# submission2019/cnn-quantization

Measured on NVIDIA H100. Metric: resnet50_w4a4_images_per_s, higher is better.
Workload: dtype f32

## Files before the change

### cnn-quantization_b200/csrc/fq_cl.cuh

```cuda
#pragma once

namespace fqb {

__device__ __forceinline__ unsigned enc_ordered(float x) {
  const unsigned b = __float_as_uint(x);
  return (b & 0x80000000u) ? ~b : (b | 0x80000000u);
}
__device__ __forceinline__ float dec_ordered(unsigned e) {
  return __uint_as_float((e & 0x80000000u) ? (e & 0x7fffffffu) : ~e);
}

constexpr unsigned kAccU = 2u * kMaxNhwcChannels;
constexpr unsigned kAccD = 3u * kMaxNhwcChannels;

struct ClView {
  unsigned* amin_inv;
  unsigned* amax;
  double* asum;
  double* asq;
  double* aabs;
};
__device__ __forceinline__ ClView cl_view(const FusedArgs& A, unsigned bank) {
  ClView v;
  v.amin_inv = A.amin_inv + bank * kAccU;
  v.amax = v.amin_inv + kMaxNhwcChannels;
  v.asum = A.asum + bank * kAccD;
  v.asq = v.asum + kMaxNhwcChannels;
  v.aabs = v.asq + kMaxNhwcChannels;
  return v;
}

__device__ __forceinline__ void red_add_f64(double* p, double v) {
  asm volatile("red.global.add.f64 [%0], %1;" ::"l"(p), "d"(v) : "memory");
}
__device__ __forceinline__ void red_max_u32(unsigned* p, unsigned v) {
  asm volatile("red.global.max.u32 [%0], %1;" ::"l"(p), "r"(v) : "memory");
}

__device__ __noinline__ void grid_arrive_cl(GridSync* gs, unsigned& epoch) {
  ++epoch;
  consumer_sync();
  if (threadIdx.x == 0) {
    unsigned prev;
    asm volatile("atom.add.acq_rel.gpu.global.u32 %0, [%1], 1;" : "=r"(prev) : "l"(&gs->arrive) : "memory");
    if (prev + 1u == epoch * gridDim.x) st_release_u32(&gs->release, epoch);
  }
}
__device__ __noinline__ void grid_wait_cl(GridSync* gs, unsigned epoch) {
  if (threadIdx.x == 0) {
    while (ld_acquire_u32(&gs->release) < epoch) __nanosleep(32);
  }
  consumer_sync();
}
__device__ __forceinline__ void grid_barrier_cl(GridSync* gs, unsigned& epoch) {
  grid_arrive_cl(gs, epoch);
  grid_wait_cl(gs, epoch);
}
__device__ __forceinline__ void grid_exit_cl(GridSync* gs) {
  consumer_sync();
  if (threadIdx.x == 0) {
    const unsigned prev = atomicAdd(&gs->exited, 1u);
    if (prev + 1u == gridDim.x) {
      gs->arrive = 0u;
      gs->release = 0u;
      for (int i = 0; i < 8; ++i) gs->unit_counter[i] = 0u;
      gs->launch_count = gs->launch_count + 1u;
      __threadfence();
      gs->exited = 0u;
    }
  }
}

constexpr unsigned kClChunkStages = 1;

struct ClStats1 {
  float mn[4], mx[4], k[4], fs[4], fq[4];
  double s[4], q[4];
  unsigned cnt;
  __device__ __forceinline__ void init(const FusedArgs& A, unsigned c0, bool active) {
    float4 first = make_float4(0.f, 0.f, 0.f, 0.f);
    if (active) first = ld_tensor(reinterpret_cast<const float4*>(A.in) + (c0 >> 2));
    k[0] = first.x;
    k[1] = first.y;
    k[2] = first.z;
    k[3] = first.w;
    cnt = 0;
#pragma unroll
    for (int i = 0; i < 4; ++i) {
      mn[i] = INFINITY;
      mx[i] = -INFINITY;
      fs[i] = 0.f;
      fq[i] = 0.f;
      s[i] = 0.0;
      q[i] = 0.0;
    }
  }
  __device__ __forceinline__ void flush() {
#pragma unroll
    for (int i = 0; i < 4; ++i) {
      s[i] += static_cast<double>(fs[i]);
      q[i] += static_cast<double>(fq[i]);
      fs[i] = 0.f;
      fq[i] = 0.f;
    }
    cnt = 0;
  }
  __device__ __forceinline__ void consume(const float4& v, unsigned) {
    const float x[4] = {v.x, v.y, v.z, v.w};
#pragma unroll
    for (int i = 0; i < 4; ++i) {
      const float d = __fsub_rn(x[i], k[i]);
      mn[i] = fminf(mn[i], x[i]);
      mx[i] = fmaxf(mx[i], x[i]);
      fs[i] = __fadd_rn(fs[i], d);
      fq[i] = __fmaf_rn(d, d, fq[i]);
    }
  }
  __device__ __forceinline__ void stage_end(const StageMeta&) {
    if (++cnt == kClChunkStages) flush();
  }
};

struct ClStats2 {
  float mu[4], bias[4], fa[4];
  double sa[4];
  unsigned cnt;
  __device__ __forceinline__ void init(const FusedArgs& A, unsigned c0, bool active, const float (&mean)[4]) {
    cnt = 0;
#pragma unroll
    for (int i = 0; i < 4; ++i) {
      bias[i] = (A.bias && active) ? __ldg(A.bias + c0 + i) : 0.f;
      mu[i] = mean[i];
      fa[i] = 0.f;
      sa[i] = 0.0;
    }
  }
  __device__ __forceinline__ void flush() {
#pragma unroll
    for (int i = 0; i < 4; ++i) {
      sa[i] += static_cast<double>(fa[i]);
      fa[i] = 0.f;
    }
    cnt = 0;
  }
  __device__ __forceinline__ void consume(const float4& v, unsigned) {
    const float x[4] = {v.x, v.y, v.z, v.w};
#pragma unroll
    for (int i = 0; i < 4; ++i) fa[i] = __fadd_rn(fa[i], fabsf(__fsub_rn(__fadd_rn(x[i], bias[i]), mu[i])));
  }
  __device__ __forceinline__ void stage_end(const StageMeta&) {
    if (++cnt == kClChunkStages) flush();
  }
};

constexpr unsigned kHistWords = 8192;
static_assert(kHistWords * 4u <= kStageBytes, "the histogram borrows one ring stage");

template <int LEAF, bool HIST>
struct ClApply {
  const FusedArgs& A;
  unsigned* hist;
  LeafParam q[4];
  float r[4], bias[4];
  unsigned nlo[4], nhi[4];
  unsigned hbase;
  bool fast;
  LeafParam rq[4];
  float rr[4], rbias[4];
  bool rquant;
  __device__ __forceinline__ void init(unsigned c0, bool active, const LeafParam (&lp)[4]) {
    fast = true;
    rquant = A.residual != nullptr && A.residual_stats != nullptr;
#pragma unroll
    for (int i = 0; i < 4; ++i) {
      rq[i].a = 1.f;
      rq[i].b = 0.f;
      rq[i].c = 0.f;
      rq[i].flags = 0;
      rr[i] = 1.f;
      rbias[i] = 0.f;
      if (rquant && active) {
        const float* row = A.residual_stats + static_cast<size_t>(c0 + i) * FQB200_STATS_STRIDE;
        rq[i].a = __ldg(row + 8);
        rq[i].b = __ldg(row + 9);
        rq[i].c = __ldg(row + 10);
        rq[i].flags = static_cast<int>(__ldg(row + 11));
        const Divisor dr = make_divisor(rq[i].a);
        rr[i] = dr.r;
        fast = fast && dr.fast;
        if (A.residual_bias) rbias[i] = __ldg(A.residual_bias + c0 + i);
      }
    }
    const unsigned copies = max(1u, min(static_cast<unsigned>(kWarps), kHistWords / static_cast<unsigned>(max(A.hist_bins, 1))));
    hbase = ((threadIdx.x >> 5) % copies) * static_cast<unsigned>(A.hist_bins);
#pragma unroll
    for (int i = 0; i < 4; ++i) {
      q[i] = lp[i];
      const Divisor dv = make_divisor(q[i].a);
      r[i] = dv.r;
      fast = fast && dv.fast;
      bias[i] = (A.bias && active) ? __ldg(A.bias + c0 + i) : 0.f;
      nlo[i] = 0u;
      nhi[i] = 0u;
    }
  }
  __device__ __forceinline__ void count(int i, float gq) {
    if (LEAF == FQB200_LEAF_MIDTREAD) {
      if (gq == q[i].c) {
        ++nhi[i];
        return;
      }
      if (gq == q[i].b) {
        ++nlo[i];
        return;
      }
    }
    if (gq == gq) {
      const float v = fminf(fmaxf(gq + static_cast<float>(A.hist_offset), 0.f), static_cast<float>(A.hist_bins - 1));
      atomicAdd(hist + hbase + static_cast<unsigned>(v), 1u);
    }
  }
  template <bool FAST, bool PAIR, bool RQ = false>
  __device__ __forceinline__ void one(const float4& v, const float4& rv, unsigned off) {
    const float x[4] = {v.x, v.y, v.z, v.w};
    float y[4], gq[4];
#pragma unroll
    for (int i = 0; i < 4; ++i) {
      Divisor dv;
      dv.s = q[i].a;
      dv.r = r[i];
      dv.fast = FAST;
      y[i] = leaf_apply<LEAF, FAST>(__fadd_rn(x[i], bias[i]), q[i], dv, 0.f, gq[i]);
    }
    if (PAIR) {
      float res[4] = {rv.x, rv.y, rv.z, rv.w};
      if (RQ) {
#pragma unroll
        for (int i = 0; i < 4; ++i) {
          Divisor dr;
          dr.s = rq[i].a;
          dr.r = rr[i];
          dr.fast = FAST;
          float g2;
          res[i] = leaf_apply<LEAF, FAST>(__fadd_rn(res[i], rbias[i]), rq[i], dr, 0.f, g2);
        }
      }
#pragma unroll
      for (int i = 0; i < 4; ++i) {
        y[i] = __fadd_rn(y[i], res[i]);
        if (A.residual_relu) y[i] = y[i] < 0.f ? 0.f : y[i];
      }
    }
    st_tensor(reinterpret_cast<float4*>(A.out) + off, make_float4(y[0], y[1], y[2], y[3]));
    if (HIST) {
#pragma unroll
      for (int i = 0; i < 4; ++i) count(i, gq[i]);
    }
  }
  __device__ __forceinline__ void consume(const float4& v, unsigned off) {
    if (fast)
      one<true, false>(v, v, off);
    else
      one<false, false>(v, v, off);
  }
  template <bool FAST>
  __device__ __forceinline__ void pooled_one(const float4& a0, const float4& a1, const float4& b0, const float4& b1, unsigned off) {
    auto mx = [](float p, float q) { return (q > p || q != q) ? q : p; };
    const float m[4] = {mx(mx(mx(a0.x, a1.x), b0.x), b1.x), mx(mx(mx(a0.y, a1.y), b0.y), b1.y),
                        mx(mx(mx(a0.z, a1.z), b0.z), b1.z), mx(mx(mx(a0.w, a1.w), b0.w), b1.w)};
    float y[4], gq;
#pragma unroll
    for (int i = 0; i < 4; ++i) {
      Divisor dv;
      dv.s = q[i].a;
      dv.r = r[i];
      dv.fast = FAST;
      y[i] = leaf_apply<LEAF, FAST>(__fadd_rn(m[i], bias[i]), q[i], dv, 0.f, gq);
    }
    st_tensor(reinterpret_cast<float4*>(A.pool_out) + off, make_float4(y[0], y[1], y[2], y[3]));
  }
  __device__ __forceinline__ void pooled(const float4& a0, const float4& a1, const float4& b0, const float4& b1, unsigned off) {
    if (fast)
      pooled_one<true>(a0, a1, b0, b1, off);
    else
      pooled_one<false>(a0, a1, b0, b1, off);
  }
  float pm[4];
  __device__ __forceinline__ void pool_begin() {
#pragma unroll
    for (int i = 0; i < 4; ++i) pm[i] = -INFINITY;
  }
  __device__ __forceinline__ void pool_tap(const float4& v) {
    auto mx = [](float p, float q) { return (q > p || q != q) ? q : p; };
    pm[0] = mx(pm[0], v.x);
    pm[1] = mx(pm[1], v.y);
    pm[2] = mx(pm[2], v.z);
    pm[3] = mx(pm[3], v.w);
  }
  template <bool FAST>
  __device__ __forceinline__ void pool_end_one(unsigned off) {
    float y[4], gq;
#pragma unroll
    for (int i = 0; i < 4; ++i) {
      Divisor dv;
      dv.s = q[i].a;
      dv.r = r[i];
      dv.fast = FAST;
      y[i] = leaf_apply<LEAF, FAST>(__fadd_rn(pm[i], bias[i]), q[i], dv, 0.f, gq);
    }
    st_tensor(reinterpret_cast<float4*>(A.pool_out) + off, make_float4(y[0], y[1], y[2], y[3]));
  }
  __device__ __forceinline__ void pool_end(unsigned off) {
    if (fast)
      pool_end_one<true>(off);
    else
      pool_end_one<false>(off);
  }
  __device__ __forceinline__ void consume2(const float4& v, const float4& rv, unsigned off) {
    if (rquant) {
      if (fast)
        one<true, true, true>(v, rv, off);
      else
        one<false, true, true>(v, rv, off);
    } else if (fast) {
      one<true, true>(v, rv, off);
    } else {
      one<false, true>(v, rv, off);
    }
  }
  __device__ __forceinline__ void stage_end(const StageMeta&) {}
};

constexpr unsigned kClItems = 4;

template <typename T, typename Op>
__device__ __forceinline__ void cl_stage_round(unsigned char* buf, unsigned cv, unsigned stride, const T (&v)[4], T identity, Op op,
                                               T (&res)[kClItems]) {
  T* st = reinterpret_cast<T*>(buf);
  consumer_sync();
#pragma unroll
  for (int i = 0; i < 4; ++i) st[i * kConsumers + threadIdx.x] = (threadIdx.x < stride) ? v[i] : identity;
  consumer_sync();
#pragma unroll
  for (unsigned k = 0; k < kClItems; ++k) {
    const unsigned it = threadIdx.x + k * kConsumers;
    T a = identity;
    if (it < 4u * cv) {
      const unsigned col = it % cv, i = it / cv;
      for (unsigned t = col; t < stride; t += cv) a = op(a, st[i * kConsumers + t]);
    }
    res[k] = a;
  }
}

__device__ __noinline__ void cl_combine_s1(unsigned char* buf, unsigned cv, unsigned stride, const unsigned (&umn)[4],
                                           const unsigned (&umx)[4], const double (&s)[4], const double (&q)[4], unsigned* dmn,
                                           unsigned* dmx, double* ds, double* dq) {
  if (cv == stride) {
    if (threadIdx.x < stride) {
#pragma unroll
      for (int i = 0; i < 4; ++i) {
        const unsigned c = 4u * threadIdx.x + i;
        red_max_u32(dmn + c, umn[i]);
        red_max_u32(dmx + c, umx[i]);
        red_add_f64(ds + c, s[i]);
        red_add_f64(dq + c, q[i]);
      }
    }
    return;
  }
  uint2 mm[4], rmm[kClItems];
#pragma unroll
  for (int i = 0; i < 4; ++i) mm[i] = make_uint2(umn[i], umx[i]);
  auto max2 = [](uint2 a, uint2 b) { return make_uint2(a.x > b.x ? a.x : b.x, a.y > b.y ? a.y : b.y); };
  double rs[kClItems], rq[kClItems];
  cl_stage_round(buf, cv, stride, mm, make_uint2(0u, 0u), max2, rmm);
  cl_stage_round(buf, cv, stride, s, 0.0, OpAdd(), rs);
  cl_stage_round(buf, cv, stride, q, 0.0, OpAdd(), rq);
#pragma unroll
  for (unsigned k = 0; k < kClItems; ++k) {
    const unsigned it = threadIdx.x + k * kConsumers;
    if (it < 4u * cv) {
      const unsigned c = 4u * (it % cv) + it / cv;
      red_max_u32(dmn + c, rmm[k].x);
      red_max_u32(dmx + c, rmm[k].y);
      red_add_f64(ds + c, rs[k]);
      red_add_f64(dq + c, rq[k]);
    }
  }
}
__device__ __noinline__ void cl_combine_add_f64(unsigned char* buf, unsigned cv, unsigned stride, const double (&v0)[4], double* d0,
                                                const double (&v1)[4], double* d1, const double (&v2)[4], double* d2) {
  if (cv == stride) {
    if (threadIdx.x < stride) {
#pragma unroll
      for (int i = 0; i < 4; ++i) {
        const unsigned c = 4u * threadIdx.x + i;
        red_add_f64(d0 + c, v0[i]);
        if (d1) red_add_f64(d1 + c, v1[i]);
        if (d2) red_add_f64(d2 + c, v2[i]);
      }
    }
    return;
  }
  double r0[kClItems], r1[kClItems], r2[kClItems];
  cl_stage_round(buf, cv, stride, v0, 0.0, OpAdd(), r0);
// ... 86 lines not shown
      A.gprior[c] = p;
      local += static_cast<double>(p);
    }
    const float psum = static_cast<float>(block_reduce(local, OpAdd(), sm.d));
    const float budget = static_cast<float>(static_cast<double>(C) * exp2(static_cast<double>(A.mt_target)));
    for (unsigned c = threadIdx.x; c < C; c += kConsumers) A.gbits[c] = rintf(__fdiv_rn(__fmul_rn(budget, A.gprior[c]), psum));
  } else {
    solve_bit_alloc(A, sm);
  }
  consumer_sync();
  if (publish && threadIdx.x == 0) st_release_u32(&A.sync->aux_ready, tag);
}

template <int LEAF, bool DEV>
__device__ __noinline__ LeafParam cl_channel_param(const FusedArgs& A, const ClView& acc, unsigned rep, unsigned C, unsigned c,
                                                   float mu, double n, bool alloc, bool do_export) {
  auto umax = [](unsigned a, unsigned b) { return a > b ? a : b; };
  const unsigned lo = cl_rep_reduce(acc.amin_inv, rep, C, c, 0u, umax);
  const unsigned hi = cl_rep_reduce(acc.amax, rep, C, c, 0u, umax);
  const double sa = DEV ? cl_rep_reduce(acc.aabs, rep, C, c, 0.0, OpAdd()) : 0.0;
  const float cb = A.bias ? __ldg(A.bias + c) : 0.f;
  const float mn = __fadd_rn(dec_ordered(~lo), cb), mx = __fadd_rn(dec_ordered(hi), cb);
  const float b = DEV ? static_cast<float>(sa / n) : 0.f;
  const bool need_sd = A.range_mode == FQB200_RANGE_GAUS || A.range_mode == FQB200_RANGE_KSTD || do_export;
  const float sd = need_sd ? cl_std(acc, rep, C, c, n) : 0.f;
  const float aux = alloc ? ld_ws(A.gbits + c) : static_cast<float>(A.num_bits);
  LeafParam q;
  if constexpr (LEAF == FQB200_LEAF_MIDTREAD) {
    float rng;
    q = mid_tread_param(A, aux, mn, mx, mu, b, rng);
    if (do_export) export_stats(A, c, mn, mx, mu, b, sd, rng, 0.f, aux, q);
  } else {
    float delta, offset;
    solve_range(A, mn, mx, mu, b, sd, aux, delta, offset);
    q = make_leaf_param(LEAF, delta, offset, aux);
    if (do_export) export_stats(A, c, mn, mx, mu, b, sd, delta, offset, aux, q);
  }
  return q;
}

struct ClCtx {
  const FlatGeo* g;
  BulkRing* ring;
  unsigned char* stages;
  unsigned char* cbuf;
  RingPos pos;
  ClView acc;
  unsigned rep_base, c0;
  bool active;
};

__device__ __noinline__ void cl_phase_s1(const FusedArgs& A, ClCtx& cx, float (&kshift)[4]) {
  const FlatGeo& g = *cx.g;
  ClStats1 s1;
  s1.init(A, cx.c0, cx.active);
#pragma unroll
  for (int i = 0; i < 4; ++i) kshift[i] = s1.k[i];
  RingPos pos = cx.pos;
  consume_phase(g, *cx.ring, cx.stages, pos, s1);
  cx.pos = pos;
  s1.flush();
  if (blockIdx.x == 0) stamp(A, 13);
  unsigned umn[4], umx[4];
#pragma unroll
  for (int i = 0; i < 4; ++i) {
    umn[i] = ~enc_ordered(s1.mn[i]);
    umx[i] = enc_ordered(s1.mx[i]);
  }
  const ClView& acc = cx.acc;
  const unsigned rb = cx.rep_base;
  cl_combine_s1(cx.cbuf, g.cv, g.stride, umn, umx, s1.s, s1.q, acc.amin_inv + rb, acc.amax + rb, acc.asum + rb, acc.asq + rb);
}

__device__ __noinline__ void cl_phase_s2(const FusedArgs& A, ClCtx& cx, const float (&mean)[4]) {
  const FlatGeo& g = *cx.g;
  ClStats2 s2;
  s2.init(A, cx.c0, cx.active, mean);
  RingPos pos = cx.pos;
  consume_phase(g, *cx.ring, cx.stages, pos, s2);
  cx.pos = pos;
  s2.flush();
  if (blockIdx.x == 0) stamp(A, 14);
  const ClView& acc = cx.acc;
  const unsigned rb = cx.rep_base;
  cl_combine_add_f64(cx.cbuf, g.cv, g.stride, s2.sa, acc.aabs + rb, s2.sa, nullptr, s2.sa, nullptr);
}

template <int LEAF, bool HIST>
__device__ __noinline__ void cl_phase_apply(const FusedArgs& A, ClCtx& cx, const LeafParam (&lp)[4], unsigned* hist) {
  const FlatGeo& g = *cx.g;
  const unsigned t = threadIdx.x;
  if (HIST) {
    for (unsigned i = t; i < kHistWords; i += kConsumers) hist[i] = 0u;
    consumer_sync();
  }
  ClApply<LEAF, HIST> ap{A, hist};
  ap.init(cx.c0, cx.active, lp);
  RingPos pos = cx.pos;
  if (A.pool.tiles) {
    if (A.pool.kind == 3u)
      consume_pool3_phase(g, A.pool, *cx.ring, cx.stages, pos, ap);
    else
      consume_pool_phase(g, A.pool, *cx.ring, cx.stages, pos, ap);
  } else if (A.residual) {
    const FlatGeo h = half_geo(g);
    consume_pair_phase(h, *cx.ring, cx.stages, pos, ap);
  } else {
    consume_phase(g, *cx.ring, cx.stages, pos, ap);
  }
  cx.pos = pos;
  if (HIST) {
    consumer_sync();
    const unsigned bins = static_cast<unsigned>(A.hist_bins);
    const unsigned copies = max(1u, min(static_cast<unsigned>(kWarps), kHistWords / bins));
    for (unsigned b = t; b < bins; b += kConsumers) {
      unsigned long long cnt = 0;
      for (unsigned w = 0; w < copies; ++w) cnt += hist[w * bins + b];
      if (cnt) atomicAdd(A.hist + b, cnt);
    }
    if (LEAF == FQB200_LEAF_MIDTREAD && A.hist_clamped && cx.active) {
#pragma unroll
      for (int i = 0; i < 4; ++i) {
        if (ap.nlo[i]) atomicAdd(A.hist_clamped + 2u * (cx.c0 + i), static_cast<unsigned long long>(ap.nlo[i]));
        if (ap.nhi[i]) atomicAdd(A.hist_clamped + 2u * (cx.c0 + i) + 1u, static_cast<unsigned long long>(ap.nhi[i]));
      }
    }
  }
}

constexpr unsigned kClStagingBytes = 4u * kConsumers * 8u;
constexpr unsigned kClTableChannels = 1024;
constexpr unsigned kClCombineBytes = kClStagingBytes + kClTableChannels * 4u;

template <int LEAF, bool DEV, bool HIST>
__global__ void __launch_bounds__(kBulkThreads, kBulkCtasPerSm) fq_cl_kernel(const __grid_constant__ FusedArgs A) {
  extern __shared__ __align__(128) unsigned char fq_dyn[];
  unsigned char* stages = fq_dyn;
  unsigned char* cbuf = fq_dyn + kStages * kStageBytes;
  float* tab_mean = reinterpret_cast<float*>(cbuf + kClStagingBytes);
  unsigned* hist = reinterpret_cast<unsigned*>(stages + (kStages - 1) * kStageBytes);
  __shared__ BulkRing ring;
  __shared__ LeaderSmem lsm;
  __shared__ alignas(8) unsigned long long solver_done;
  const FlatGeo& g = A.flat;
  const unsigned C = g.channels, cv = g.cv;
  const unsigned launch = ld_ws(&A.sync->launch_count);
  const unsigned bank = launch & 1u;
  const unsigned tag = launch + 1u;
  const bool alloc = (LEAF == FQB200_LEAF_MIDTREAD) || (A.bit_alloc && A.num_bits <= 4);
  const bool aux_needs_b = alloc && LEAF != FQB200_LEAF_MIDTREAD && A.prior == FQB200_PRIOR_B;
  const bool solver_in_s2 = alloc && !aux_needs_b && DEV && gridDim.x > 1u;
  __shared__ alignas(8) unsigned long long phase_go[2];
  if (threadIdx.x == 0) {
    mbar_init(smem_u32(&solver_done), 1u);
    mbar_init(smem_u32(&phase_go[0]), 1u);
    mbar_init(smem_u32(&phase_go[1]), 1u);
  }
  const unsigned nstages = HIST ? kStages - 1u : kStages;
  ring_init(ring, nstages);

  if (threadIdx.x >= kConsumers) {
    if (threadIdx.x == kConsumers) {
      RingPos pos;
      pos.init(nstages);
      const float4* src = reinterpret_cast<const float4*>(A.in);
      const TicketPlan all = {2u, blockIdx.x, gridDim.x, 2u * gridDim.x};
      const TicketPlan no0 = {blockIdx.x == 0 ? 0u : 2u, blockIdx.x - 1u, gridDim.x - 1u, 2u * (gridDim.x - 1u)};
      produce_phase<false>(g, src, &A.sync->unit_counter[0], all, ring, stages, pos);
      if (DEV) {
        mbar_wait(smem_u32(&phase_go[0]), 0u);
        if (solver_in_s2 && blockIdx.x == 0) mbar_wait(smem_u32(&solver_done), 0u);
        produce_phase<true>(g, src, &A.sync->unit_counter[1], solver_in_s2 ? no0 : all, ring, stages, pos);
      }
      if (!A.stats_only) {
        mbar_wait(smem_u32(&phase_go[1]), 0u);
        if (A.pool.tiles && A.pool.kind == 3u)
          produce_pool3_phase(g, A.pool, src, &A.sync->unit_counter[2], all, ring, stages, pos);
        else if (A.pool.tiles)
          produce_pool_phase(g, A.pool, src, &A.sync->unit_counter[2], all, ring, stages, pos);
        else if (A.residual)
          produce_phase<!DEV, true>(half_geo(g), src, &A.sync->unit_counter[2], all, ring, stages, pos,
                                    reinterpret_cast<const float4*>(A.residual));
        else
          produce_phase<!DEV>(g, src, &A.sync->unit_counter[2], all, ring, stages, pos);
      }
    }
    return;
  }

  const unsigned t = threadIdx.x;
  const bool active = t < g.stride;
  const bool direct = cv == g.stride;
  const unsigned col = active ? t % cv : 0u;
  const unsigned c0 = 4u * col;
  const double n = A.n_per_group;
  const ClView acc = cl_view(A, bank);
  const unsigned rep = A.nhwc_rep;
  const unsigned rep_base = (blockIdx.x % rep) * C;
  unsigned epoch = 0;
  if (blockIdx.x == 0) stamp(A, 0);

  if (blockIdx.x == gridDim.x - 1u) {
    const ClView other = cl_view(A, bank ^ 1u);
    uint4* zu = reinterpret_cast<uint4*>(other.amin_inv);
    uint4* zd = reinterpret_cast<uint4*>(other.asum);
    const uint4 z = make_uint4(0u, 0u, 0u, 0u);
    for (unsigned i = t; i < kAccU / 4u; i += kConsumers) zu[i] = z;
    for (unsigned i = t; i < kAccD / 2u; i += kConsumers) zd[i] = z;
  }

  ClCtx cx;
  cx.g = &g;
  cx.ring = &ring;
  cx.stages = stages;
  cx.cbuf = cbuf;
  cx.pos.init(nstages);
  cx.acc = acc;
  cx.rep_base = rep_base;
  cx.c0 = c0;
  cx.active = active;
  float kshift[4];
  cl_phase_s1(A, cx, kshift);
  if (t == 0) mbar_arrive(smem_u32(&phase_go[DEV ? 0 : 1]));
  if (blockIdx.x == 0) stamp(A, 1);
  grid_barrier_cl(A.sync, epoch);
  if (blockIdx.x == 0) stamp(A, 4);

  float mean[4];
  if (direct) {
#pragma unroll
    for (int i = 0; i < 4; ++i)
      mean[i] = static_cast<float>(cl_mean(acc, rep, C, c0 + i, kshift[i], (A.bias && active) ? __ldg(A.bias + c0 + i) : 0.f, n));
  } else {
    for (unsigned c = t; c < C; c += kConsumers)
      tab_mean[c] = static_cast<float>(cl_mean(acc, rep, C, c, ld_tensor(A.in + c), A.bias ? __ldg(A.bias + c) : 0.f, n));
    consumer_sync();
#pragma unroll
    for (int i = 0; i < 4; ++i) mean[i] = tab_mean[c0 + i];
  }

  if (alloc && !aux_needs_b && blockIdx.x == 0) {
    cl_solve_aux(A, acc, lsm, tag, false, !solver_in_s2);
    stamp(A, 12);
    if (t == 0) mbar_arrive(smem_u32(&solver_done));
  }

  if constexpr (DEV) {
    cl_phase_s2(A, cx, mean);
    if (t == 0) mbar_arrive(smem_u32(&phase_go[1]));
    if (blockIdx.x == 0) stamp(A, 5);
    grid_barrier_cl(A.sync, epoch);
    if (blockIdx.x == 0) stamp(A, 8);
    if (aux_needs_b && blockIdx.x == 0) cl_solve_aux(A, acc, lsm, tag, true, true);
  }
  if (alloc && !solver_in_s2) {
    if (t == 0)
      while (ld_acquire_u32(&A.sync->aux_ready) != tag) __nanosleep(40);
    consumer_sync();
  }

  LeafParam lp[4];
  const bool do_export = A.out_stats != nullptr && blockIdx.x == 0;
  if (direct) {
#pragma unroll
    for (int i = 0; i < 4; ++i) lp[i] = cl_channel_param<LEAF, DEV>(A, acc, rep, C, c0 + i, mean[i], n, alloc, do_export && active);
  } else {
    LeafParam* tab_lp = reinterpret_cast<LeafParam*>(cbuf);
    consumer_sync();
    for (unsigned c = t; c < C; c += kConsumers) tab_lp[c] = cl_channel_param<LEAF, DEV>(A, acc, rep, C, c, tab_mean[c], n, alloc, do_export);
    consumer_sync();
#pragma unroll
    for (int i = 0; i < 4; ++i) lp[i] = tab_lp[c0 + i];
  }
  if (blockIdx.x == 0) stamp(A, 7);

  if (!A.stats_only) {
    cl_phase_apply<LEAF, HIST>(A, cx, lp, hist);
    if (blockIdx.x == 0) stamp(A, 9);
  }
  grid_exit_cl(A.sync);
}

template <bool GRID>
struct ClGiven {
  const FusedArgs& A;
  LeafParam q[4];
  float r[4], bias[4];
  bool fast;
  template <bool FAST>
  __device__ __forceinline__ void one(const float4& v, unsigned off) {
    const float x[4] = {v.x, v.y, v.z, v.w};
    float y[4], gq[4];
#pragma unroll
    for (int i = 0; i < 4; ++i) {
      Divisor dv;
      dv.s = q[i].a;
      dv.r = r[i];
      dv.fast = FAST;
      y[i] = leaf_apply<FQB200_LEAF_TORCH, FAST>(__fadd_rn(x[i], bias[i]), q[i], dv, 0.f, gq[i]);
    }
    st_tensor(reinterpret_cast<float4*>(A.out) + off, make_float4(y[0], y[1], y[2], y[3]));
    if (GRID) st_tensor(reinterpret_cast<float4*>(A.grid_out) + off, make_float4(gq[0], gq[1], gq[2], gq[3]));
  }
  __device__ __forceinline__ void consume(const float4& v, unsigned off) {
    if (fast)
      one<true>(v, off);
    else
      one<false>(v, off);
  }
  __device__ __forceinline__ void stage_end(const StageMeta&) {}
};

template <bool GRID>
__global__ void __launch_bounds__(kBulkThreads, kBulkCtasPerSm) fq_cl_given_kernel(const __grid_constant__ FusedArgs A) {
  extern __shared__ __align__(128) unsigned char fq_dyn[];
  __shared__ BulkRing ring;
  const FlatGeo& g = A.flat;
  ring_init(ring);
  if (threadIdx.x >= kConsumers) {
    if (threadIdx.x == kConsumers) {
      RingPos pos;
      pos.init();
      const TicketPlan tp = {0xffffffffu, blockIdx.x, gridDim.x, 0u};
      produce_phase<false>(g, reinterpret_cast<const float4*>(A.in), nullptr, tp, ring, fq_dyn, pos);
    }
    return;
  }
  const unsigned t = threadIdx.x;
  const bool active = t < g.stride;
  const unsigned c0 = active ? 4u * (t % g.cv) : 0u;
  ClGiven<GRID> ap{A};
  ap.fast = true;
#pragma unroll
  for (int i = 0; i < 4; ++i) {
    const unsigned c = c0 + i;
    const unsigned pi = A.given_per_group ? c : 0u;
    const float bits = A.g_bits ? __ldg(A.g_bits + c) : static_cast<float>(A.num_bits);
    ap.q[i] = make_leaf_param(FQB200_LEAF_TORCH, __ldg(A.g_delta + pi), __ldg(A.g_offset + pi), bits);
    const Divisor dv = make_divisor(ap.q[i].a);
    ap.r[i] = dv.r;
    ap.fast = ap.fast && dv.fast;
    ap.bias[i] = (A.bias && active) ? __ldg(A.bias + c) : 0.f;
  }
  RingPos pos;
  pos.init();
  consume_phase(g, ring, fq_dyn, pos, ap);
}

__global__ void __launch_bounds__(kBulkThreads, kBulkCtasPerSm) fq_cl_given_fused_kernel(const __grid_constant__ FusedArgs A) {
  extern __shared__ __align__(128) unsigned char fq_dyn[];
  __shared__ BulkRing ring;
  const FlatGeo& g = A.flat;
  ring_init(ring);
  if (threadIdx.x >= kConsumers) {
    if (threadIdx.x == kConsumers) {
      RingPos pos;
      pos.init();
      const float4* src = reinterpret_cast<const float4*>(A.in);
      const TicketPlan tp = {0xffffffffu, blockIdx.x, gridDim.x, 0u};
      if (A.pool.tiles && A.pool.kind == 3u)
        produce_pool3_phase(g, A.pool, src, nullptr, tp, ring, fq_dyn, pos);
      else if (A.pool.tiles)
        produce_pool_phase(g, A.pool, src, nullptr, tp, ring, fq_dyn, pos);
      else if (A.residual)
        produce_phase<false, true>(half_geo(g), src, nullptr, tp, ring, fq_dyn, pos, reinterpret_cast<const float4*>(A.residual));
      else
        produce_phase<false>(g, src, nullptr, tp, ring, fq_dyn, pos);
    }
    return;
  }
  const unsigned t = threadIdx.x;
  const bool active = t < g.stride;
  const unsigned c0 = active ? 4u * (t % g.cv) : 0u;
  LeafParam lp[4];
#pragma unroll
  for (int i = 0; i < 4; ++i) {
    const unsigned c = c0 + i;
    const float bits = A.g_bits ? __ldg(A.g_bits + c) : static_cast<float>(A.num_bits);
    lp[i] = make_leaf_param(FQB200_LEAF_TORCH, __ldg(A.g_delta + c), __ldg(A.g_offset + c), bits);
  }
  ClApply<FQB200_LEAF_TORCH, false> ap{A, nullptr};
  ap.init(c0, active, lp);
  RingPos pos;
  pos.init();
  if (A.pool.tiles && A.pool.kind == 3u)
    consume_pool3_phase(g, A.pool, ring, fq_dyn, pos, ap);
  else if (A.pool.tiles)
    consume_pool_phase(g, A.pool, ring, fq_dyn, pos, ap);
  else if (A.residual)
    consume_pair_phase(half_geo(g), ring, fq_dyn, pos, ap);
  else
    consume_phase(g, ring, fq_dyn, pos, ap);
}

struct LeafBulkArgs {
  FlatGeo flat;
  const float* in;
  float* out;
  const float* noise;
  LeafParam q;
};

template <bool NOISE>
struct LeafBulk {
  const LeafBulkArgs& A;
  Divisor dv;
  template <bool FAST>
  __device__ __forceinline__ void one(const float4& v, const float4& nz, unsigned off) {
    float gq;
    float4 y;
    y.x = leaf_apply<FQB200_LEAF_COMPILED, FAST, NOISE>(v.x, A.q, dv, NOISE ? nz.x : 0.f, gq);
    y.y = leaf_apply<FQB200_LEAF_COMPILED, FAST, NOISE>(v.y, A.q, dv, NOISE ? nz.y : 0.f, gq);
    y.z = leaf_apply<FQB200_LEAF_COMPILED, FAST, NOISE>(v.z, A.q, dv, NOISE ? nz.z : 0.f, gq);
    y.w = leaf_apply<FQB200_LEAF_COMPILED, FAST, NOISE>(v.w, A.q, dv, NOISE ? nz.w : 0.f, gq);
    st_tensor(reinterpret_cast<float4*>(A.out) + off, y);
  }
  __device__ __forceinline__ void consume(const float4& v, unsigned off) {
    if (dv.fast)
      one<true>(v, v, off);
    else
      one<false>(v, v, off);
  }
  __device__ __forceinline__ void consume2(const float4& v, const float4& nz, unsigned off) {
    if (dv.fast)
      one<true>(v, nz, off);
    else
      one<false>(v, nz, off);
  }
  __device__ __forceinline__ void stage_end(const StageMeta&) {}
};

template <bool NOISE>
__global__ void __launch_bounds__(kBulkThreads, kBulkCtasPerSm) fq_leaf_bulk_kernel(const __grid_constant__ LeafBulkArgs A) {
// ... 445 lines not shown
```

### cnn-quantization_b200/csrc/fqb200.cu

```cuda
#include <cuda_runtime.h>
#include <math.h>
#include <stdint.h>
#include <stdio.h>
#include <stdlib.h>
#include <string.h>

#include "../../include/fqb200.h"
#include "fq_device.cuh"
#include "fq_bulk.cuh"

namespace fqb {

__constant__ float kGaus[9] = {0.f, 1.24f, 1.71f, 2.15f, 2.55f, 2.93f, 3.28f, 3.61f, 3.92f};
__constant__ float kGausPos[9] = {0.f, 1.71f, 2.15f, 2.55f, 2.93f, 3.28f, 3.61f, 3.92f, 4.2f};
__constant__ float kLaplace[9] = {1.05f, 1.86f, 2.83f, 3.89f, 5.03f, 6.2f, 7.41f, 8.64f, 9.89f};
__constant__ float kLaplacePos[9] = {1.86f, 2.83f, 3.89f, 5.02f, 6.2f, 7.41f, 8.64f, 9.89f, 11.16f};
constexpr int kTable = 101;
__constant__ double kOmegaTable[kTable];
__constant__ double kAlphaTable[kTable];

enum : int { FLAG_PASSTHROUGH = 1, FLAG_TRUE_ZERO = 2, FLAG_RELU = 4 };

struct alignas(16) LeafParam {
  float a, b, c;
// ... 1244 lines not shown
      continue;
    }
    if (worst < 1) {
      d.rc = FQB200_ERR_CUDA;
      snprintf(d.err, sizeof(d.err), "channels-last kernel does not fit on an SM");
      return;
    }
    d.resident_cl[hist] = sms * worst;
  }
  {
    int n = 0;
    const void* fn = reinterpret_cast<const void*>(fqb::fq_cl_bca_kernel);
    e = cudaFuncSetAttribute(fn, cudaFuncAttributeMaxDynamicSharedMemorySize, static_cast<int>(cl_smem(false)));
    if (e == cudaSuccess) e = cudaOccupancyMaxActiveBlocksPerMultiprocessor(&n, fn, fqb::kBulkThreads, cl_smem(false));
    if (e != cudaSuccess || n < 1) return bad("bias-correction kernel setup", e);
    d.resident_bca = sms * n;
  }
  {
    int n = 0;
    const void* fn = reinterpret_cast<const void*>(fqb::fq_rows_kernel);
    e = cudaFuncSetAttribute(fn, cudaFuncAttributeMaxDynamicSharedMemorySize, static_cast<int>(cl_given_smem()));
    if (e == cudaSuccess) e = cudaOccupancyMaxActiveBlocksPerMultiprocessor(&n, fn, fqb::kBulkThreads, cl_given_smem());
    if (e != cudaSuccess || n < 1) return bad("row kernel setup", e);
    d.resident_rows = sms * n;
  }
  const void* given[4] = {reinterpret_cast<const void*>(fqb::fq_given_kernel<4, FQB200_LEAF_TORCH, false>),
                          reinterpret_cast<const void*>(fqb::fq_given_kernel<4, FQB200_LEAF_TORCH, true>),
                          reinterpret_cast<const void*>(fqb::fq_cl_given_kernel<false>),
                          reinterpret_cast<const void*>(fqb::fq_cl_given_kernel<true>)};
  for (int i = 0; i < 4; ++i) {
    e = cudaFuncSetAttribute(given[i], cudaFuncAttributeMaxDynamicSharedMemorySize,
                             static_cast<int>(i < 2 ? dyn_smem(4) : cl_given_smem()));
    if (e != cudaSuccess) return bad("given-parameter kernel setup", e);
  }
  e = cudaFuncSetAttribute(reinterpret_cast<const void*>(fqb::fq_cl_given_fused_kernel), cudaFuncAttributeMaxDynamicSharedMemorySize,
                           static_cast<int>(cl_given_smem()));
  if (e != cudaSuccess) return bad("given-parameter fused kernel setup", e);
  const void* leafb[2] = {reinterpret_cast<const void*>(fqb::fq_leaf_bulk_kernel<false>),
                          reinterpret_cast<const void*>(fqb::fq_leaf_bulk_kernel<true>)};
  for (int i = 0; i < 2; ++i) {
    e = cudaFuncSetAttribute(leafb[i], cudaFuncAttributeMaxDynamicSharedMemorySize, static_cast<int>(cl_given_smem()));
    if (e != cudaSuccess) return bad("a1 bulk kernel setup", e);
  }
  double om[fqb::kTable], al[fqb::kTable];
  om[0] = 0.0;
  al[0] = 0.0;
  const double lo[5] = {0.01, 0.1, 1, 10, 100}, hi[5] = {0.1, 1, 10, 100, 1000};
  for (int dcd = 0; dcd < 5; ++dcd)
    for (int k = 0; k < 20; ++k) {
      const double w = lo[dcd] + (hi[dcd] - lo[dcd]) * k / 20.0;
      om[1 + dcd * 20 + k] = w;
      al[1 + dcd * 20 + k] = laplace_opt_alpha(w);
    }
  e = cudaMemcpyToSymbol(fqb::kOmegaTable, om, sizeof(om));
  if (e == cudaSuccess) e = cudaMemcpyToSymbol(fqb::kAlphaTable, al, sizeof(al));
  if (e != cudaSuccess) return bad("table upload", e);
  d.sms = sms;
  d.resident = sms * per_sm;
}

int get_device(DeviceInfo** out) {
  int dev = 0;
  cudaError_t e = cudaGetDevice(&dev);
  if (e != cudaSuccess) return fail(FQB200_ERR_CUDA, "cudaGetDevice: %s", cudaGetErrorString(e));
  if (dev < 0 || dev >= kMaxDevices) return fail(FQB200_ERR_UNSUPPORTED, "device index out of range%s");
  std::call_once(g_dev_once[dev], init_device, dev);
  DeviceInfo& d = g_dev[dev];
  if (d.rc != FQB200_OK) return fail(d.rc, "device set-up failed: %s", d.err);
  *out = &d;
  return FQB200_OK;
}

struct Plan {
  fqb::Geometry geo;
  fqb::FlatGeo flat;
  int vec;
  int mode;
  int grid;
};

bool aligned16(const void* p) { return (reinterpret_cast<uintptr_t>(p) & 15u) == 0; }

constexpr uint64_t kUnitsPerCta = 8;

int make_plan(int64_t outer, int64_t groups, int64_t inner, bool can_vec, bool allow_bundle, int max_ctas, Plan* pl) {
  if (outer <= 0 || groups <= 0 || inner <= 0) return fail(FQB200_ERR_INVALID, "non-positive tensor extent%s");
  if (groups > 0x3fffffffLL || outer > 0x7fffffffLL || inner > 0x7fffffffLL * 4LL)
    return fail(FQB200_ERR_UNSUPPORTED, "tensor extent exceeds 2^31%s");
  int vec = (can_vec && inner % 4 == 0) ? 4 : 1;
  int mode = vec;
  uint64_t bundle = 1;
  if (vec == 1 && can_vec && allow_bundle && inner >= 4) {
    const uint64_t b = (inner % 2 == 0) ? 2 : 4;
    const uint64_t row_v = b * static_cast<uint64_t>(inner) / 4;
    if (groups % b == 0 && row_v <= static_cast<uint64_t>(fqb::kThreads)) {
      bundle = b;
      vec = 4;
      mode = 8;
    }
  }
  const uint64_t G = static_cast<uint64_t>(groups) / bundle;
  const uint64_t inner_v = bundle * static_cast<uint64_t>(inner) / vec;
  if (inner_v > 0xffffffffULL) return fail(FQB200_ERR_UNSUPPORTED, "row too long%s");
  const uint64_t stride = (mode == 8) ? (fqb::kThreads / inner_v) * inner_v : fqb::kThreads;
  const uint64_t group_v = static_cast<uint64_t>(outer) * inner_v;
  const uint64_t total_v = group_v * G;
  if (total_v >= (1ULL << 32)) return fail(FQB200_ERR_UNSUPPORTED, "tensors of 2^32 vectors (64 GB) and more are not supported%s");
  const uint64_t ctas = static_cast<uint64_t>(max_ctas);
  const uint64_t min_unit_v = static_cast<uint64_t>(fqb::kRingDepth) * stride;
  uint64_t parts = (kUnitsPerCta * ctas + G - 1) / G;
  const uint64_t max_parts = group_v / min_unit_v > 0 ? group_v / min_unit_v : 1;
  if (parts > max_parts) parts = max_parts;
  if (parts < 1) parts = 1;
  while ((group_v + parts - 1) / parts >= 0x7fffffffULL) ++parts;
  uint64_t part_v = (group_v + parts - 1) / parts;
  if (mode == 8) part_v = (part_v + inner_v - 1) / inner_v * inner_v;
  parts = (group_v + part_v - 1) / part_v;
  if (parts * G >= 0xfffffff0ULL) return fail(FQB200_ERR_UNSUPPORTED, "too many work units%s");
  const uint64_t units = parts * G;
  unsigned lanes = 32;
  while (lanes > 1 && (static_cast<uint64_t>(fqb::kThreads / lanes) < static_cast<uint64_t>(groups) || (lanes >> 1) >= parts)) lanes >>= 1;
  fqb::Geometry& g = pl->geo;
  g.groups = static_cast<unsigned>(G);
  g.channels = static_cast<unsigned>(groups);
  g.bundle = static_cast<unsigned>(bundle);
  g.stride = static_cast<unsigned>(stride);
  g.parts = static_cast<unsigned>(parts);
  g.units = static_cast<unsigned>(units);
  g.inner_v = static_cast<unsigned>(inner_v);
  g.step_q = static_cast<unsigned>(stride / inner_v);
  g.step_r = static_cast<unsigned>(stride % inner_v);
  g.red_lanes = lanes;
  g.part_v = static_cast<unsigned>(part_v);
  g.group_v = group_v;
  g.row_pitch = G * inner_v;
  pl->vec = vec;
  pl->mode = mode;
  pl->grid = static_cast<int>(units < ctas ? units : ctas);
  return FQB200_OK;
}

bool flat_eligible(int64_t channels) { return channels % 4 == 0 && channels / 4 >= 1 && channels / 4 <= fqb::kConsumers; }

int make_plan_flat(uint64_t elems, int64_t channels, int max_ctas, Plan* pl) {
  if (elems == 0 || elems % 4 != 0) return fail(FQB200_ERR_UNSUPPORTED, "flat stream needs a multiple of 4 elements%s");
  const uint64_t total_v = elems / 4;
  if (total_v >= (1ULL << 32)) return fail(FQB200_ERR_UNSUPPORTED, "tensors of 2^32 vectors (64 GB) and more are not supported%s");
  const uint64_t cv = channels > 0 ? static_cast<uint64_t>(channels) / 4 : 1;
  if (channels > 0 && !flat_eligible(channels)) return fail(FQB200_ERR_UNSUPPORTED, "channels-last needs C %% 4 == 0 and C <= 2048%s");
  const uint64_t stride = (fqb::kConsumers / cv) * cv;
  const uint64_t stage_v = static_cast<uint64_t>(fqb::kStageVec) * stride;
  const uint64_t n_stages = (total_v + stage_v - 1) / stage_v;
  const uint64_t ctas = static_cast<uint64_t>(max_ctas);
  uint64_t unit_stages = n_stages / (kUnitsPerCta * ctas);
  if (unit_stages < 2) unit_stages = 2;
  if (unit_stages > 64) unit_stages = 64;
  const uint64_t units = (n_stages + unit_stages - 1) / unit_stages;
  fqb::FlatGeo& g = pl->flat;
  g.total_v = static_cast<unsigned>(total_v);
  g.stride = static_cast<unsigned>(stride);
  g.stage_v = static_cast<unsigned>(stage_v);
  g.n_stages = static_cast<unsigned>(n_stages);
  g.unit_stages = static_cast<unsigned>(unit_stages);
  g.units = static_cast<unsigned>(units);
  g.channels = static_cast<unsigned>(channels > 0 ? channels : 0);
  g.cv = static_cast<unsigned>(cv);
  memset(&pl->geo, 0, sizeof(pl->geo));
  pl->geo.channels = g.channels;
  pl->vec = 4;
  pl->mode = 2;
  pl->grid = static_cast<int>(units < ctas ? units : ctas);
  return FQB200_OK;
}

int make_plan_rows(uint64_t rows, uint64_t row_elems, int64_t channels, int max_ctas, Plan* pl, fqb::RowsGeo* rg) {
  if (rows == 0 || row_elems == 0 || row_elems % 4 != 0 || rows > fqb::kMaxNhwcChannels)
    return fail(FQB200_ERR_UNSUPPORTED, "row stream needs rows <= 4096 of a multiple of 4 elements%s");
  const uint64_t row_v = row_elems / 4;
  if (rows * row_v >= (1ULL << 32)) return fail(FQB200_ERR_UNSUPPORTED, "tensors of 2^32 vectors (64 GB) and more are not supported%s");
  const uint64_t cv = channels > 0 ? static_cast<uint64_t>(channels) / 4 : 1;
  if (channels > 0 && (!flat_eligible(channels) || row_v % cv != 0)) return fail(FQB200_ERR_UNSUPPORTED, "bias period does not fit the rows%s");
  const uint64_t stride = (fqb::kConsumers / cv) * cv;
  const uint64_t stage_v = static_cast<uint64_t>(fqb::kStageVec) * stride;
  const uint64_t spr = (row_v + stage_v - 1) / stage_v;
  const uint64_t ctas = static_cast<uint64_t>(max_ctas);
  uint64_t unit_stages = rows * spr / (kUnitsPerCta * ctas);
  if (unit_stages < 1) unit_stages = 1;
  if (unit_stages > 64) unit_stages = 64;
  if (unit_stages > spr) unit_stages = spr;
  const uint64_t upr = (spr + unit_stages - 1) / unit_stages;
  const uint64_t units = rows * upr;
  if (units >= 0xfffffff0ULL) return fail(FQB200_ERR_UNSUPPORTED, "too many work units%s");
  fqb::FlatGeo& g = pl->flat;
  g.total_v = static_cast<unsigned>(rows * row_v);
  g.stride = static_cast<unsigned>(stride);
  g.stage_v = static_cast<unsigned>(stage_v);
  g.n_stages = static_cast<unsigned>(rows * spr);
  g.unit_stages = static_cast<unsigned>(unit_stages);
  g.units = static_cast<unsigned>(units);
  g.channels = static_cast<unsigned>(channels > 0 ? channels : 0);
  g.cv = static_cast<unsigned>(cv);
  rg->rows = static_cast<unsigned>(rows);
  rg->row_v = static_cast<unsigned>(row_v);
  rg->stages_per_row = static_cast<unsigned>(spr);
  rg->units_per_row = static_cast<unsigned>(upr);
  memset(&pl->geo, 0, sizeof(pl->geo));
  pl->geo.channels = static_cast<unsigned>(rows);
  pl->vec = 4;
  pl->mode = 3;
  pl->grid = static_cast<int>(units < ctas ? units : ctas);
  return FQB200_OK;
}

bool rows_supported(const fqb200_desc* d, bool can_vec) {
  if (d->leaf != FQB200_LEAF_COMPILED || d->range_mode != FQB200_RANGE_MINMAX || d->bias_corr || d->var_corr || d->channels_last ||
      d->out_hist || !can_vec || d->outer != 1 || d->inner % 4 != 0 || d->groups > static_cast<int64_t>(fqb::kMaxNhwcChannels))
    return false;
  if (!(d->scope == FQB200_SCOPE_GROUP_MEAN || d->scope == FQB200_SCOPE_TENSOR || d->groups == 1)) return false;
  if (d->bias) {
    if (d->bias_period >= 0) return false;
    const int64_t c = -d->bias_period;
    if (!flat_eligible(c) || d->inner % c != 0) return false;
  }
  return true;
}

size_t align_up(size_t v, size_t a) { return (v + a - 1) / a * a; }

size_t carve(char* base, uint64_t slots, uint64_t groups, fqb::FusedArgs* A) {
  size_t off = 0;
  auto take = [&](size_t bytes) {
    char* p = base ? base + off : nullptr;
    off = align_up(off + bytes, 256);
    return p;
  };
  char* sync = take(sizeof(fqb::GridSync));
  char* acc_u = take(2 * fqb::kAccU * sizeof(unsigned));
  char* acc_d = take(2 * fqb::kAccD * sizeof(double));
  char* pmin = take(slots * sizeof(float));
  char* pmax = take(slots * sizeof(float));
  char* psum = take((slots + 2 * groups) * sizeof(double));
  char* pabs = take((slots + 2 * groups) * sizeof(double));
  char* psq = take((slots + 2 * groups) * sizeof(double));
  char* gf = take(groups * sizeof(float) * 12);
  char* gd = take(groups * sizeof(double));
  char* lp = take(groups * sizeof(fqb::LeafParam));
  if (A) {
    A->sync = reinterpret_cast<fqb::GridSync*>(sync);
    A->pmin = reinterpret_cast<float*>(pmin);
    A->pmax = reinterpret_cast<float*>(pmax);
    A->psum = reinterpret_cast<double*>(psum);
    A->pabs = reinterpret_cast<double*>(pabs);
    A->psq = reinterpret_cast<double*>(psq);
    float* f = reinterpret_cast<float*>(gf);
    A->gmin = f + 0 * groups;
    A->gmax = f + 1 * groups;
    A->gmean = f + 2 * groups;
    A->gb = f + 3 * groups;
    A->gstd = f + 4 * groups;
    A->gbits = f + 5 * groups;
    A->gprior = f + 6 * groups;
    A->gdelta = f + 7 * groups;
    A->goffset = f + 8 * groups;
    A->cq = f + 9 * groups;
    A->co = f + 10 * groups;
    A->ck = f + 11 * groups;
    A->gmean_d = reinterpret_cast<double*>(gd);
    A->lp = reinterpret_cast<fqb::LeafParam*>(lp);
    A->amin_inv = reinterpret_cast<unsigned*>(acc_u);
    A->amax = nullptr;
    A->asum = reinterpret_cast<double*>(acc_d);
    A->aabs = nullptr;
    A->asq = nullptr;
  }
  return off;
}

int check_desc(const fqb200_desc* d) {
  if (!d) return fail(FQB200_ERR_INVALID, "null descriptor%s");
  if (d->scope < FQB200_SCOPE_GROUP || d->scope > FQB200_SCOPE_TENSOR) return fail(FQB200_ERR_INVALID, "bad scope%s");
  if (d->range_mode < FQB200_RANGE_MINMAX || d->range_mode > FQB200_RANGE_GIVEN) return fail(FQB200_ERR_INVALID, "bad range_mode%s");
  if (d->range_mode == FQB200_RANGE_GIVEN &&
      (!d->channels_last || d->leaf != FQB200_LEAF_TORCH || d->scope != FQB200_SCOPE_GROUP || d->stats_only || d->out_stats || d->out_hist ||
       d->bias_corr || d->var_corr || d->bit_alloc || !d->given_delta || !d->given_offset))
    return fail(FQB200_ERR_UNSUPPORTED, "RANGE_GIVEN: channels_last, torch leaf, scope GROUP, given_delta / given_offset, no statistics outputs%s");
  if (d->leaf < FQB200_LEAF_TORCH || d->leaf > FQB200_LEAF_MIDTREAD) return fail(FQB200_ERR_INVALID, "bad leaf%s");
  if (d->leaf != FQB200_LEAF_MIDTREAD && (d->num_bits < 1 || d->num_bits > 8))
    return fail(FQB200_ERR_INVALID, "num_bits must be in 1..8%s");
  if (d->scope != FQB200_SCOPE_GROUP && (d->range_mode != FQB200_RANGE_MINMAX || d->leaf == FQB200_LEAF_MIDTREAD))
    return fail(FQB200_ERR_UNSUPPORTED, "group-mean / tensor scopes are defined for min/max ranges only%s");
  if (d->bit_alloc && !(d->bit_alloc_target > 0.f)) return fail(FQB200_ERR_INVALID, "bit_alloc_target must be > 0%s");
  if ((d->bias_corr || d->var_corr) && d->scope == FQB200_SCOPE_GROUP_MEAN)
    return fail(FQB200_ERR_UNSUPPORTED, "weight correction is per row (scope GROUP or TENSOR)%s");
  return FQB200_OK;
}

bool cl_supported(const fqb200_desc* d) {
  return d->scope == FQB200_SCOPE_GROUP && d->leaf != FQB200_LEAF_COMPILED && !d->bias_corr && !d->var_corr && d->bias_period <= 0 &&
         flat_eligible(d->groups);
}
bool cl_needs_b(const fqb200_desc* d) {
  const bool alloc = d->bit_alloc && d->num_bits <= 4 && d->leaf != FQB200_LEAF_MIDTREAD;
  return d->range_mode == FQB200_RANGE_LAPLACE || (d->leaf == FQB200_LEAF_MIDTREAD && d->mt_clip) ||
         (alloc && d->bit_alloc_prior == FQB200_PRIOR_B) || d->stats_only || d->out_stats != nullptr;
}

}

extern "C" {
// ... 485 lines not shown
```

Measured before the change: 7622.

## Alternate pass direction, keep output head in L2, fix unit size, add timer probes

The first statistics pass now runs in reverse order, and the second runs forward, so each pass begins on data the previous pass left in L2. The apply phase always streams in one fixed direction, and output vectors in the first 16 MB are stored with L2-caching stores instead of streaming stores. The work-unit size is fixed at two stages rather than scaled with tensor size, which gives finer load balance at the cost of more ticket atomics. Globaltimer debug stamps are also added, gated on a debug pointer.

Result: faster. 7720 (median of 6 runs) (+1.3%).

```diff
diff --git a/cnn-quantization_b200/csrc/fq_cl.cuh b/cnn-quantization_b200/csrc/fq_cl.cuh
--- a/cnn-quantization_b200/csrc/fq_cl.cuh
+++ b/cnn-quantization_b200/csrc/fq_cl.cuh
@@ -37,10 +37,33 @@
   asm volatile("red.global.max.u32 [%0], %1;" ::"l"(p), "r"(v) : "memory");
 }
 
-__device__ __noinline__ void grid_arrive_cl(GridSync* gs, unsigned& epoch) {
+__device__ __forceinline__ unsigned long long globaltimer() {
+  unsigned long long t;
+  asm volatile("mov.u64 %0, %globaltimer;" : "=l"(t));
+  return t;
+}
+__device__ __forceinline__ unsigned long long* dbg_slot(const FusedArgs& A, int slot) { return A.dbg ? A.dbg + slot : nullptr; }
+__device__ __forceinline__ void stamp_latest(unsigned long long* dbg) {
+  if (dbg) atomicMax(dbg, globaltimer());
+}
+__device__ __forceinline__ void stamp_earliest(unsigned long long* dbg) {
+  if (dbg) atomicMin(dbg, globaltimer());
+}
+__device__ __forceinline__ void stamp_cta0(const FusedArgs& A, int slot) {
+  if (A.dbg && blockIdx.x == 0) A.dbg[slot] = globaltimer();
+}
+__device__ __forceinline__ void stamp_stage_ready(const FusedArgs& A, BulkRing& r, const RingPos& pos, int slot) {
+  if (A.dbg && blockIdx.x == 0 && threadIdx.x == 0) {
+    mbar_wait(smem_u32(&r.full[pos.slot]), pos.parity);
+    A.dbg[slot] = globaltimer();
+  }
+}
+
+__device__ __noinline__ void grid_arrive_cl(GridSync* gs, unsigned& epoch, unsigned long long* dbg = nullptr) {
   ++epoch;
   consumer_sync();
   if (threadIdx.x == 0) {
+    stamp_latest(dbg);
     unsigned prev;
     asm volatile("atom.add.acq_rel.gpu.global.u32 %0, [%1], 1;" : "=r"(prev) : "l"(&gs->arrive) : "memory");
     if (prev + 1u == epoch * gridDim.x) st_release_u32(&gs->release, epoch);
@@ -52,13 +75,14 @@
   }
   consumer_sync();
 }
-__device__ __forceinline__ void grid_barrier_cl(GridSync* gs, unsigned& epoch) {
-  grid_arrive_cl(gs, epoch);
+__device__ __forceinline__ void grid_barrier_cl(GridSync* gs, unsigned& epoch, unsigned long long* dbg = nullptr) {
+  grid_arrive_cl(gs, epoch, dbg);
   grid_wait_cl(gs, epoch);
 }
-__device__ __forceinline__ void grid_exit_cl(GridSync* gs) {
+__device__ __forceinline__ void grid_exit_cl(GridSync* gs, unsigned long long* dbg = nullptr) {
   consumer_sync();
   if (threadIdx.x == 0) {
+    stamp_latest(dbg);
     const unsigned prev = atomicAdd(&gs->exited, 1u);
     if (prev + 1u == gridDim.x) {
       gs->arrive = 0u;
@@ -155,6 +179,15 @@
 
 constexpr unsigned kHistWords = 8192;
 static_assert(kHistWords * 4u <= kStageBytes, "the histogram borrows one ring stage");
+
+constexpr unsigned kL2KeepVec = (16u << 20) / 16u;
+__device__ __forceinline__ void st_out(float* out, unsigned off, const float4& v) {
+  float4* p = reinterpret_cast<float4*>(out) + off;
+  if (off < kL2KeepVec)
+    __stcg(p, v);
+  else
+    st_tensor(p, v);
+}
 
 template <int LEAF, bool HIST>
 struct ClApply {
@@ -251,7 +284,7 @@
         if (A.residual_relu) y[i] = y[i] < 0.f ? 0.f : y[i];
       }
     }
-    st_tensor(reinterpret_cast<float4*>(A.out) + off, make_float4(y[0], y[1], y[2], y[3]));
+    st_out(A.out, off, make_float4(y[0], y[1], y[2], y[3]));
     if (HIST) {
 #pragma unroll
       for (int i = 0; i < 4; ++i) count(i, gq[i]);
@@ -644,6 +677,8 @@
   const bool solver_in_s2 = alloc && !aux_needs_b && DEV && gridDim.x > 1u;
   __shared__ alignas(8) unsigned long long phase_go[2];
   if (threadIdx.x == 0) {
+    stamp_earliest(dbg_slot(A, 16));
+    stamp_latest(dbg_slot(A, 17));
     mbar_init(smem_u32(&solver_done), 1u);
     mbar_init(smem_u32(&phase_go[0]), 1u);
     mbar_init(smem_u32(&phase_go[1]), 1u);
@@ -658,23 +693,33 @@
       const float4* src = reinterpret_cast<const float4*>(A.in);
       const TicketPlan all = {2u, blockIdx.x, gridDim.x, 2u * gridDim.x};
       const TicketPlan no0 = {blockIdx.x == 0 ? 0u : 2u, blockIdx.x - 1u, gridDim.x - 1u, 2u * (gridDim.x - 1u)};
-      produce_phase<false>(g, src, &A.sync->unit_counter[0], all, ring, stages, pos);
+      const bool s1_rev = DEV && !A.pool.tiles;
+      stamp_cta0(A, 21);
+      if (s1_rev)
+        produce_phase<true>(g, src, &A.sync->unit_counter[0], all, ring, stages, pos);
+      else
+        produce_phase<false>(g, src, &A.sync->unit_counter[0], all, ring, stages, pos);
       if (DEV) {
         mbar_wait(smem_u32(&phase_go[0]), 0u);
         if (solver_in_s2 && blockIdx.x == 0) mbar_wait(smem_u32(&solver_done), 0u);
-        produce_phase<true>(g, src, &A.sync->unit_counter[1], solver_in_s2 ? no0 : all, ring, stages, pos);
+        stamp_cta0(A, 22);
+        if (s1_rev)
+          produce_phase<false>(g, src, &A.sync->unit_counter[1], solver_in_s2 ? no0 : all, ring, stages, pos);
+        else
+          produce_phase<true>(g, src, &A.sync->unit_counter[1], solver_in_s2 ? no0 : all, ring, stages, pos);
       }
       if (!A.stats_only) {
         mbar_wait(smem_u32(&phase_go[1]), 0u);
+        stamp_cta0(A, 23);
         if (A.pool.tiles && A.pool.kind == 3u)
           produce_pool3_phase(g, A.pool, src, &A.sync->unit_counter[2], all, ring, stages, pos);
         else if (A.pool.tiles)
           produce_pool_phase(g, A.pool, src, &A.sync->unit_counter[2], all, ring, stages, pos);
         else if (A.residual)
-          produce_phase<!DEV, true>(half_geo(g), src, &A.sync->unit_counter[2], all, ring, stages, pos,
+          produce_phase<true, true>(half_geo(g), src, &A.sync->unit_counter[2], all, ring, stages, pos,
                                     reinterpret_cast<const float4*>(A.residual));
         else
-          produce_phase<!DEV>(g, src, &A.sync->unit_counter[2], all, ring, stages, pos);
+          produce_phase<true>(g, src, &A.sync->unit_counter[2], all, ring, stages, pos);
       }
     }
     return;
@@ -712,10 +757,11 @@
   cx.c0 = c0;
   cx.active = active;
   float kshift[4];
+  stamp_stage_ready(A, ring, cx.pos, 24);
   cl_phase_s1(A, cx, kshift);
   if (t == 0) mbar_arrive(smem_u32(&phase_go[DEV ? 0 : 1]));
   if (blockIdx.x == 0) stamp(A, 1);
-  grid_barrier_cl(A.sync, epoch);
+  grid_barrier_cl(A.sync, epoch, dbg_slot(A, 18));
   if (blockIdx.x == 0) stamp(A, 4);
 
   float mean[4];
@@ -738,10 +784,11 @@
   }
 
   if constexpr (DEV) {
+    stamp_stage_ready(A, ring, cx.pos, 25);
     cl_phase_s2(A, cx, mean);
     if (t == 0) mbar_arrive(smem_u32(&phase_go[1]));
     if (blockIdx.x == 0) stamp(A, 5);
-    grid_barrier_cl(A.sync, epoch);
+    grid_barrier_cl(A.sync, epoch, dbg_slot(A, 19));
     if (blockIdx.x == 0) stamp(A, 8);
     if (aux_needs_b && blockIdx.x == 0) cl_solve_aux(A, acc, lsm, tag, true, true);
   }
@@ -767,10 +814,11 @@
   if (blockIdx.x == 0) stamp(A, 7);
 
   if (!A.stats_only) {
+    stamp_stage_ready(A, ring, cx.pos, 26);
     cl_phase_apply<LEAF, HIST>(A, cx, lp, hist);
     if (blockIdx.x == 0) stamp(A, 9);
   }
-  grid_exit_cl(A.sync);
+  grid_exit_cl(A.sync, dbg_slot(A, 20));
 }
 
 template <bool GRID>
diff --git a/cnn-quantization_b200/csrc/fqb200.cu b/cnn-quantization_b200/csrc/fqb200.cu
--- a/cnn-quantization_b200/csrc/fqb200.cu
+++ b/cnn-quantization_b200/csrc/fqb200.cu
@@ -1420,9 +1420,7 @@
   const uint64_t stage_v = static_cast<uint64_t>(fqb::kStageVec) * stride;
   const uint64_t n_stages = (total_v + stage_v - 1) / stage_v;
   const uint64_t ctas = static_cast<uint64_t>(max_ctas);
-  uint64_t unit_stages = n_stages / (kUnitsPerCta * ctas);
-  if (unit_stages < 2) unit_stages = 2;
-  if (unit_stages > 64) unit_stages = 64;
+  const uint64_t unit_stages = 2;
   const uint64_t units = (n_stages + unit_stages - 1) / unit_stages;
   fqb::FlatGeo& g = pl->flat;
   g.total_v = static_cast<unsigned>(total_v);
```
